# NVlabs/curobo

Hardware: NVIDIA H100
Metric: rollout_cost_grad_evals_per_sec (higher is better)
Workload: dtype f32

## Files before the change

curobo_b200/csrc/cb200_kernels.cu:

```cuda
#include <cuda_runtime.h>
#include <stdio.h>
#include <stdlib.h>
#include <string.h>

#include <algorithm>
#include <cmath>
#include <vector>

#include "../../include/curobo_b200.h"
#include "cb200_blob.h"
#include "cb200_bspline.cuh"
#include "cb200_dynamics.cuh"
#include "cb200_dynamics_tile.cuh"
#include "cb200_launch.h"
#include "cb200_math.cuh"
#include "cb200_mesh.cuh"
#include "cb200_warp.cuh"

using namespace cb200;

namespace {

constexpr int kWarpsPerCta = 8;
constexpr int kMinCtas = 2;
// ... 70 lines not shown
  } else if (s.degree == 5) {
    st = bspline::evaluate<5>(bspline::make_polygon<5>(s.knots, b, d, D, s.n_knots, dt, s.steps, implicit, s.sp, s.sv, s.sa, s.sj, srow, s.gp, s.gv, s.ga, s.gj, grow), h, s.steps);
  } else {
    st = bspline::evaluate<4>(bspline::make_polygon<4>(s.knots, b, d, D, s.n_knots, dt, s.steps, implicit, s.sp, s.sv, s.sa, s.sj, srow, s.gp, s.gv, s.ga, s.gj, grow), h, s.steps);
  }
  return st;
}

template <bool SPLINE>
__device__ __forceinline__ bspline::State4 load_row_state(const FusedArgs &a, int e, int b, int h, int d, int D) {
  if (SPLINE) {
    const bspline::State4 st = spline_row_state(a.spl, b, h, d, D);
    const size_t idx = (size_t)e * D + d;
    if (a.spl.out_p) a.spl.out_p[idx] = st.p;
    if (a.spl.out_v) a.spl.out_v[idx] = st.v;
    if (a.spl.out_a) a.spl.out_a[idx] = st.a;
    if (a.spl.out_j) a.spl.out_j[idx] = st.j;
    return st;
  }
  const size_t idx = (size_t)e * D + d;
  bspline::State4 st;
  st.p = __ldg(a.q + idx);
  st.v = a.vel ? __ldg(a.vel + idx) : 0.0f;
  st.a = a.acc ? __ldg(a.acc + idx) : 0.0f;
  st.j = a.jerk ? __ldg(a.jerk + idx) : 0.0f;
  return st;
}

__device__ __forceinline__ float seed_dt(const FusedArgs &a, int b) {
  if (a.spl.knots != nullptr) return __ldg(a.spl.traj_dt + __ldg(a.spl.goal_idx + b));
  return a.dt ? __ldg(a.dt + b) : 1.0f;
}

__device__ __forceinline__ float cspace_dof(const FusedArgs &a, const RobotView &rv, int e, int b, int h, int d,
                                            const bspline::State4 &st, float &gp) {
  const float qd = st.p;
  const cb200_rollout_cfg &c = a.cfg;
  const int D = rv.D;
  const float *lim = rv.limits;
  float cost = 0.0f;
  gp = 0.0f;
  if (c.cspace_type == 1) {
    bound_cost(qd, lim[d], lim[D + d], c.cspace_activation[0], c.cspace_weight[0], cost, gp);
    cspace_target_term(a, b, h, d, D, qd, cost, gp);
  } else if (c.cspace_type == 2) {
    const size_t idx = (size_t)e * D + d;
    const float dt = seed_dt(a, b);
    float wb[5], wr[5];
#pragma unroll
    for (int i = 0; i < 5; ++i) {
      wb[i] = c.cspace_weight[i];
      wr[i] = c.cspace_reg[i];
    }
    const float dt2 = dt * dt, dt3 = dt2 * dt;
    if (c.retime_weights) {
      wb[1] = dt * wb[1];
      wb[2] = dt2 * wb[2];
      wb[3] = dt3 * wb[3];
    }
    if (c.retime_regularization_weights) {
      wr[0] = dt * wr[0];
      wr[1] = dt2 * wr[1];
      wr[2] = dt3 * wr[2];
      wr[4] = dt * wr[4];
    }
    const float v = st.v, ac = st.a, jk = st.j;
    float gv = 0.0f, ga = 0.0f, gj = 0.0f;
    bound_cost(qd, lim[d], lim[D + d], c.cspace_activation[0], wb[0], cost, gp);
    bound_cost(v, lim[2 * D + d], lim[3 * D + d], c.cspace_activation[1], wb[1], cost, gv);
    bound_cost(ac, lim[4 * D + d], lim[5 * D + d], c.cspace_activation[2], wb[2], cost, ga);
    bound_cost(jk, lim[6 * D + d], lim[7 * D + d], c.cspace_activation[3], wb[3], cost, gj);
    cspace_target_term(a, b, h, d, D, qd, cost, gp);
    l2_reg(v, wr[0], cost, gv);
    l2_reg(ac, wr[1], cost, ga);
    l2_reg(jk, wr[2], cost, gj);
    if (a.grad_vel) a.grad_vel[idx] = gv;
    if (a.grad_acc) a.grad_acc[idx] = ga;
    if (a.grad_jerk) a.grad_jerk[idx] = gj;
  }
  return cost;
}

template <bool SPLINE, int W = 32>
__device__ __forceinline__ void row_phase_a(const FusedArgs &a, const RobotView &rv, const EvalSmem &es, int lane, int e,
                                            int b, int h, float &cs_cost, float &pose_c) {
  const cb200_rollout_cfg &cfg = a.cfg;
  const int D = rv.D, S = rv.S, L = rv.L;
  cs_cost = 0.0f;
  #pragma unroll 1
  for (int d = lane; d < D; d += W) {
    const bspline::State4 st = load_row_state<SPLINE>(a, e, b, h, d, D);
    es.qv[d] = st.p;
    float gp;
    const float c = cspace_dof(a, rv, e, b, h, d, st, gp);
    es.gqv[d] = gp;
    cs_cost += c;
    if (a.cspace_cost) a.cspace_cost[(size_t)e * D + d] = c;
  }
  row_sync<W>();
  warp_fk<W>(rv, es, lane);
  warp_spheres<W>(rv, es, lane, a.robot_spheres ? reinterpret_cast<float4 *>(a.robot_spheres) + (size_t)e * S : nullptr,
                  row_sphere_cfg(a, b, S));
  pose_c = 0.0f;
  const bool do_pose = (a.goal_position != nullptr);
  #pragma unroll 1
  for (int t = lane; t < L; t += W) {
    const float *T = es.cumul + 12 * rv.tool_map[t];
    const V3 p = mk3(T[3], T[7], T[11]);
    const Q4 qt = quat_from_transform(T);
    if (a.link_pos) {
      float *o = a.link_pos + ((size_t)e * L + t) * 3;
      o[0] = p.x;
      o[1] = p.y;
      o[2] = p.z;
    }
    if (a.link_quat) *reinterpret_cast<float4 *>(a.link_quat + ((size_t)e * L + t) * 4) = make_float4(qt.w, qt.x, qt.y, qt.z);
    float *pg = es.pose_g + 8 * t;
    pg[0] = pg[1] = pg[2] = pg[4] = pg[5] = pg[6] = 0.0f;
    if (do_pose) {
      const int gi = a.idxs_goal ? __ldg(a.idxs_goal + b) : 0;
      const bool term = !(h < a.H - 1 && a.H > 1);
      const float *axes = term ? a.pose_axes_t : a.pose_axes_nt;
      const float *tol = term ? a.pose_tol_t : a.pose_tol_nt;
      const size_t go = ((size_t)gi * L + t) * cfg.num_goalset;
      const PoseOut po = tool_pose_cost(p, qt, a.goal_position + go * 3, a.goal_quat + go * 4, cfg.num_goalset,
                                        cfg.pose_weight[0], cfg.pose_weight[1], axes, t,
                                        tol != nullptr ? __ldg(tol + 2 * t) : 0.0f,
                                        tol != nullptr ? __ldg(tol + 2 * t + 1) : 0.0f, cfg.pose_rotation_method);
      const V3 om = quat_grad_to_omega(qt, po.gq_w, po.gq_x, po.gq_y, po.gq_z);
      pg[0] = po.g_pos.x;
      pg[1] = po.g_pos.y;
      pg[2] = po.g_pos.z;
      pg[4] = om.x;
      pg[5] = om.y;
      pg[6] = om.z;
      pose_c += po.pos_cost + po.rot_cost;
      if (a.pose_cost) {
        a.pose_cost[((size_t)e * L + t) * 2] = po.pos_cost;
        a.pose_cost[((size_t)e * L + t) * 2 + 1] = po.rot_cost;
      }
      if (a.pose_goalset_idx) a.pose_goalset_idx[(size_t)e * L + t] = po.goal_idx;
    }
  }
  row_sync<W>();
}

struct RowB1 {
  float self_c, fmax, scene_c;
  int bi, bj, nnz;
};

__device__ __forceinline__ float4 mesh_terms(const MeshSet *ms, float eta, float w, V3 c, float r, int env, bool sweep, bool has_prev,
                                          V3 prev, bool has_next, V3 next) {
  const CuboidSet no_cuboids{};
  const VoxelSet no_voxels{};
  V3 g = mk3(0, 0, 0);
  const float cost = sweep ? sphere_scene_swept<4>(c, r, eta, w, has_prev, prev, has_next, next, no_cuboids, no_voxels, env, g, ms)
                           : sphere_scene_discrete<4>(c, r, eta, w, no_cuboids, no_voxels, env, g, ms);
  return make_float4(g.x, g.y, g.z, cost);
}

template <bool SWEEP, int SCENE, bool CULL2 = true, int W = 32>
__device__ __forceinline__ RowB1 row_phase_b1(const FusedArgs &a, const RobotView &rv, const EvalSmem &es, int lane, int e,
                                              int b, const float4 *prev_sph, const float4 *next_sph) {
  const cb200_rollout_cfg &cfg = a.cfg;
  const int S = rv.S;
  RowB1 r{0.0f, 0.0f, 0.0f, 0, 0, 0};
  if (cfg.self_weight > 0.0f && rv.P > 0) {
    r.fmax = (rv.n_lp > 0) ? warp_self_collision_tiles<true, CULL2, W>(rv, es, lane, r.bi, r.bj)
                           : warp_self_collision_pairs<W>(es.gsph, rv.pairs, rv.P, lane, r.bi, r.bj);
    r.self_c = (r.fmax > 0.0f) ? 0.5f * cfg.self_weight * r.fmax : 0.0f;
  }
  if (a.self_cost && lane == 0) a.self_cost[e] = r.self_c;
  row_sync<W>();
  const bool do_scene = SCENE != 0 && cfg.scene_weight > 0.0f;
  const int env = (a.env_query_idx != nullptr) ? __ldg(a.env_query_idx + b) : 0;
  const float sdt = (SWEEP && cfg.use_speed_metric && (a.dt != nullptr || a.spl.knots != nullptr))
                        ? (a.spl.knots != nullptr ? __ldg(a.spl.traj_dt + __ldg(a.spl.goal_idx)) : __ldg(a.dt))
                        : 0.0f;
  int ce = 0, ncub = 0;
  bool cull = false;
  if ((SCENE & 1) && do_scene && (!(SCENE & 4) || a.cuboids.inv_pose != nullptr)) {
    ce = env < a.cuboids.num_envs ? env : 0;
    ncub = a.cuboids.count[ce];
    if (ncub > a.cuboids.max_n) ncub = a.cuboids.max_n;
    cull = !SWEEP && rv.n_lp > 0 && ncub <= 32;
    if (cull) {
#pragma unroll 1
      for (int ca = lane; ca < rv.n_cl; ca += W) {
        const float4 cb = rv.cl_bound_scene[ca];
        uint32_t mask = 0u;
        if (cb.w >= 0.0f) {
          const float *Tk = es.cumul + 12 * rv.cl_link[ca];
          const V3 cw = mk3(Tk[0] * cb.x + Tk[1] * cb.y + Tk[2] * cb.z + Tk[3], Tk[4] * cb.x + Tk[5] * cb.y + Tk[6] * cb.z + Tk[7],
                            Tk[8] * cb.x + Tk[9] * cb.y + Tk[10] * cb.z + Tk[11]);
#pragma unroll 1
          for (int i = 0; i < ncub; ++i) {
            const int kk = ce * a.cuboids.max_n + i;
            if (a.cuboids.enable[kk] != 1) continue;
            const ObsFrame f = load_obs_frame(a.cuboids.inv_pose + 8 * kk);
            const SdfGrad sg = cuboid_sdf_grad(to_obstacle(f, cw), ldgf(a.cuboids.dims + 4 * kk), ldgf(a.cuboids.dims + 4 * kk + 1),
                                               ldgf(a.cuboids.dims + 4 * kk + 2));
            if (sg.sdf < cb.w + cfg.scene_activation) mask |= (1u << i);
          }
        }
        es.cmask[ca] = mask;
      }
      row_sync<W>();
    }
// ... 36 lines not shown
            const float4 m = mesh_terms(&a.meshes, cfg.scene_activation, cfg.scene_weight, cen, sp.w, env, false, false, cen, false, cen);
            c += m.w;
            g = g + mk3(m.x, m.y, m.z);
          }
        }
      } else {
        V3 pv = cen, nx = cen;
        if (prev_sph != nullptr) {
          const float4 t = prev_sph[s];
          pv = mk3(t.x, t.y, t.z);
        }
        if (next_sph != nullptr) {
          const float4 t = next_sph[s];
          nx = mk3(t.x, t.y, t.z);
        }
        c = sphere_scene_swept<SCENE & 3>(cen, sp.w, cfg.scene_activation, cfg.scene_weight, prev_sph != nullptr, pv,
                                          next_sph != nullptr, nx, a.cuboids, a.voxels, env, g);
        if (SCENE & 4) {
          const float4 m = mesh_terms(&a.meshes, cfg.scene_activation, cfg.scene_weight, cen, sp.w, env, true, prev_sph != nullptr,
                                      pv, next_sph != nullptr, nx);
          c += m.w;
          g = g + mk3(m.x, m.y, m.z);
        }
        if (cfg.use_speed_metric && prev_sph != nullptr && next_sph != nullptr) speed_metric(pv, cen, nx, sdt, c, g);
      }
    }
    es.gsph[s] = make_float4(g.x, g.y, g.z, 0.0f);
    r.nnz += (g.x != 0.0f || g.y != 0.0f || g.z != 0.0f) ? 1 : 0;
    r.scene_c += c;
    if (a.scene_cost) a.scene_cost[(size_t)e * S + s] = c;
  }
  row_sync<W>();
  r.nnz = (int)row_reduce<W, 0>((unsigned)r.nnz) + 2;
  return r;
}

template <bool SMALL = false, int W = 32>
__device__ __forceinline__ void row_phase_b2(const FusedArgs &a, const RobotView &rv, const EvalSmem &es,
                                             const unsigned char *smem_blob, int lane, int e, const RowB1 &r,
                                             float cs_cost, float pose_c) {
  if (r.fmax > 0.0f && lane == 0) {
    const float4 pi = es.sph[r.bi], pj = es.sph[r.bj];
    const float w = a.cfg.self_weight;
    float4 gi = es.gsph[r.bi], gj = es.gsph[r.bj];
    const float gx = w * (pj.x - pi.x), gy = w * (pj.y - pi.y), gz = w * (pj.z - pi.z);
    gi.x += gx;
    gi.y += gy;
    gi.z += gz;
    gj.x -= gx;
    gj.y -= gy;
    gj.z -= gz;
    es.gsph[r.bi] = gi;
    es.gsph[r.bj] = gj;
  }
  row_sync<W>();
  float *gq = a.grad_q + (size_t)e * rv.D;
  if (!warp_fk_backward_sparse<SMALL, W>(rv, es, lane, gq, r.nnz)) warp_fk_backward_cold<W>(smem_blob, a.blob, es.cumul, lane, gq);
  const float tot = warp_sum<W>(cs_cost + pose_c + r.scene_c) + r.self_c;
  if (lane == 0) a.cost[e] = tot;
  row_sync<W>();
}

template <int SCENE, bool SPLINE, int MINB = kMinCtas, int ROWS = 1>
__global__ void __launch_bounds__(kWarpsPerCta * 32, MINB) rollout_fused_kernel(const __grid_constant__ FusedArgs a) {
  static_assert(ROWS == 1 || (ROWS == 2 && MINB == 3 && !SPLINE), "paired rows: arm build only");
  constexpr int W = 32 / ROWS;
  CB200_EXTERN_SHARED __align__(128) unsigned char smem[];
  __shared__ unsigned long long mbar;
  stage_blob_to_smem(smem, a.blob, (uint32_t)a.blob_smem_bytes, &mbar);
  const int warp = threadIdx.x >> 5, lane = threadIdx.x & (W - 1), nwarps = blockDim.x >> 5;
  const int half = ROWS == 1 ? 0 : (int)(threadIdx.x >> 4) & 1;
  const bool leader = (threadIdx.x & 31) == 0;
  float *base = reinterpret_cast<float *>(smem + a.blob_smem_bytes) + (size_t)(warp * ROWS + half) * a.eval_floats;
  const int N = a.B * a.H;
  const int stride = gridDim.x * nwarps;
  int u = blockIdx.x * nwarps + warp;
  while (u * ROWS < N) {
    const int e = u * ROWS + half;
    if (ROWS == 1 || e < N) {
      int b = e, h = 0;
      if (a.H != 1) {
        b = e / a.H;
        h = e - b * a.H;
      }
      const RobotView rv = make_robot_view(smem, a.blob);
      const EvalSmem es = carve_eval_smem(base, rv.nl, rv.D, rv.S, rv.L, rv.n_cl);
      float cs_cost = 0.0f, pose_c = 0.0f;
      row_phase_a<SPLINE, W>(a, rv, es, lane, e, b, h, cs_cost, pose_c);
      const RowB1 r = row_phase_b1<false, SCENE, MINB != 3, W>(a, rv, es, lane, e, b, nullptr, nullptr);
      row_phase_b2<MINB == 3, W>(a, rv, es, smem, lane, e, r, cs_cost, pose_c);
    }
    if (a.work_counter != nullptr) {
      int nxt = 0;
      if (leader) nxt = stride + atomicAdd(a.work_counter, 1);
      u = __shfl_sync(kFull, nxt, 0);
    } else {
      u += stride;
    }
  }
  if (a.work_counter != nullptr && leader) {
    __threadfence();
    if (atomicAdd(a.work_counter + 1, 1) == stride - 1) {
      a.work_counter[0] = 0;
      a.work_counter[1] = 0;
    }
  }
}

constexpr int kBigWarps = 16;

template <int SCENE, bool SMALL = false>
__device__ __forceinline__ RowB1 row_phase_b1_list(const FusedArgs &a, const RobotView &rv, const EvalSmem &es, int lane, int e,
                                                   int b, int &n_list, bool &dense) {
  const cb200_rollout_cfg &cfg = a.cfg;
  const int S = rv.S;
  RowB1 r{0.0f, 0.0f, 0.0f, 0, 0, 0};
  n_list = 0;
  dense = false;
  if (cfg.self_weight > 0.0f && rv.P > 0) {
    r.fmax = warp_self_collision_tiles<false, !SMALL>(rv, es, lane, r.bi, r.bj);
    r.self_c = (r.fmax > 0.0f) ? 0.5f * cfg.self_weight * r.fmax : 0.0f;
  }
  if (a.self_cost && lane == 0) a.self_cost[e] = r.self_c;
  __syncwarp();
  const bool do_scene = SCENE != 0 && cfg.scene_weight > 0.0f;
  const int env = (a.env_query_idx != nullptr) ? __ldg(a.env_query_idx + b) : 0;
  int ce = 0, ncub = 0;
  bool cull = false;
  if ((SCENE & 1) && do_scene && (!(SCENE & 4) || a.cuboids.inv_pose != nullptr)) {
    ce = env < a.cuboids.num_envs ? env : 0;
    ncub = a.cuboids.count[ce];
    if (ncub > a.cuboids.max_n) ncub = a.cuboids.max_n;
// ... 1422 lines not shown
      if (d > best) {
        best = d;
        arg = i;
      }
    }
    return best;
  };
  int arg;
  double best_R = farthest(c, arg), best_c[3] = {c[0], c[1], c[2]};
  for (int it = 1; it <= 200; ++it) {
    const double R = farthest(c, arg);
    if (R < best_R) {
      best_R = R;
      for (int k = 0; k < 3; ++k) best_c[k] = c[k];
    }
    const double dx = bx[arg] - c[0], dy = by[arg] - c[1], dz = bz[arg] - c[2];
    const double d = std::sqrt(dx * dx + dy * dy + dz * dz);
    if (d < 1e-12) break;
    const double mv = std::min(R / (it + 1.0), d) / d;
    c[0] += dx * mv;
    c[1] += dy * mv;
    c[2] += dz * mv;
  }
  const double Rf = farthest(best_c, arg);
  out[0] = (float)best_c[0];
  out[1] = (float)best_c[1];
  out[2] = (float)best_c[2];
  double cr[3] = {(double)out[0], (double)out[1], (double)out[2]};
  const double Rr = farthest(cr, arg);
  out[3] = (float)(std::max(Rf, Rr) * (1.0 + 1e-4) + 1e-5);
}

static thread_local int g_last_variant = 0;

extern "C" {

int cb200_abi_version(void) { return CB200_ABI_VERSION; }
int cb200_last_rollout_variant(void) { return g_last_variant; }
int cb200_sm_arch(void) { return 90; }
const char *cb200_error_string(int err) { return cudaGetErrorString((cudaError_t)err); }

int cb200_device_info(int device, int *sm_count, int *max_smem_optin) {
  cudaError_t e = cudaDeviceGetAttribute(sm_count, cudaDevAttrMultiProcessorCount, device);
  if (e != cudaSuccess) return ret(e);
  return ret(cudaDeviceGetAttribute(max_smem_optin, cudaDevAttrMaxSharedMemoryPerBlockOptin, device));
}

int cb200_kinematics_forward_spheres(float *link_pos, float *link_quat, float *batch_robot_spheres,
                                     float *batch_center_of_mass, float *global_cumul_mat, const float *joint_vec,
                                     const float *fixed_transform, const float *robot_spheres,
                                     const float *link_masses_com, const int8_t *joint_map_type,
                                     const int16_t *joint_map, const int16_t *link_map, const int16_t *tool_frame_map,
                                     const int16_t *link_sphere_map, const float *joint_offset_map,
                                     const int32_t *env_query_idx, int num_envs, int batch_size, int horizon,
                                     int n_joints, int num_spheres, int num_links, int n_tool_frames,
                                     int write_global_cumul, int compute_com, cb200_stream_t stream) {
  CB200_DEVICE_GUARD(joint_vec);
  if (batch_size < 0 || num_links < 1 || horizon < 1) return ret(cudaErrorInvalidValue);
  if (compute_com != 0 && (batch_center_of_mass == nullptr || link_masses_com == nullptr)) return ret(cudaErrorInvalidValue);
  if (batch_size == 0) return ret(cudaSuccess);
  KinFwdArgs a{link_pos, link_quat, batch_robot_spheres, global_cumul_mat, joint_vec, fixed_transform, robot_spheres,
               joint_offset_map, joint_map_type, joint_map, link_map, tool_frame_map, link_sphere_map, env_query_idx,
               num_envs, batch_size, horizon, n_joints, num_spheres, num_links, n_tool_frames, write_global_cumul,
               link_masses_com, batch_center_of_mass};
  const size_t smem = (size_t)kWarpsPerCta * num_links * 12 * sizeof(float);
  void (*kern)(const KinFwdArgs) = compute_com != 0 ? kin_forward_kernel<true> : kin_forward_kernel<false>;
  if (smem > 48 * 1024) {
    cudaError_t e = cudaFuncSetAttribute(kern, cudaFuncAttributeMaxDynamicSharedMemorySize, (int)smem);
    if (e != cudaSuccess) return ret(e);
  }
  const int grid = persistent_grid(kern, kWarpsPerCta * 32, smem, (batch_size + kWarpsPerCta - 1) / kWarpsPerCta);
// ... 408 lines not shown
          lps.push_back((uint32_t)a | ((uint32_t)b << 16));
          covered += (long long)(cl_start[a + 1] - cl_start[a]) * (cl_start[b + 1] - cl_start[b]);
        }
      }
      ok = ok && covered == P && (int)lps.size() <= lp_cap(sz);
    }
    if (ok) {
      std::sort(lps.begin(), lps.end(), [](uint32_t x, uint32_t y) {
        return ((x & 0xffffu) != (y & 0xffffu)) ? (x & 0xffffu) < (y & 0xffffu) : (x >> 16) < (y >> 16);
      });
      BlobHeader *hh = reinterpret_cast<BlobHeader *>(o);
      hh->n_cl = n_cl;
      hh->n_lp = (int32_t)lps.size();
      int16_t *cll = reinterpret_cast<int16_t *>(o + h.off_cl_link);
      int16_t *cls = reinterpret_cast<int16_t *>(o + h.off_cl_start);
      float *clb = reinterpret_cast<float *>(o + h.off_cl_bound);
      for (int a = 0; a < n_cl; ++a) {
        cll[a] = (int16_t)cl_link[a];
        cls[a] = (int16_t)cl_start[a];
        bounding_ball(link_spheres, sphere_padding, cl_start[a], cl_start[a + 1], clb + 4 * a, n_cfg, S);
        bounding_ball(link_spheres, nullptr, cl_start[a], cl_start[a + 1],
                      reinterpret_cast<float *>(o + h.off_cl_bound_scene) + 4 * a, n_cfg, S);
      }
      cls[n_cl] = (int16_t)S;
      memcpy(o + h.off_lp, lps.data(), lps.size() * 4);
      for (int s0 = 0; s0 < S; ++s0) o[h.off_sph_cl + s0] = (unsigned char)cl_of_sphere[s0];
    }
  }
  return total;
}

int cb200_rollout_cost_grad(const cb200_rollout_cfg *cfg, const cb200_rollout_io *io, cb200_stream_t stream) {
  CB200_DEVICE_GUARD((io != nullptr ? io->cost : nullptr));
  if (cfg == nullptr || io == nullptr || io->robot_blob == nullptr || io->cost == nullptr || io->grad_q == nullptr ||
      io->batch_size < 0 || io->horizon < 1)
    return ret(cudaErrorInvalidValue);
  const cb200_spline_input *sp = io->spline;
  if (sp == nullptr && io->q == nullptr) return ret(cudaErrorInvalidValue);
  int spline_steps = 0;
  if (sp != nullptr) {
    if (sp->knots == nullptr || sp->start_position == nullptr || sp->start_velocity == nullptr ||
        sp->start_acceleration == nullptr || sp->start_jerk == nullptr || sp->start_idx == nullptr ||
        sp->goal_idx == nullptr || sp->traj_dt == nullptr || sp->use_implicit_goal_state == nullptr ||
        sp->goal_position == nullptr || sp->goal_velocity == nullptr || sp->goal_acceleration == nullptr ||
        sp->goal_jerk == nullptr || sp->n_knots < 1 || sp->degree < 3 || sp->degree > 5)
      return ret(cudaErrorInvalidValue);
    spline_steps = (io->horizon - 1) / (sp->n_knots + sp->degree + 1);
    if (sp->grad_knots != nullptr &&
        (io->grad_vel == nullptr || io->grad_acc == nullptr || io->grad_jerk == nullptr || io->horizon - 1 < 5 ||
         spline_steps < 1 || spline_steps > 32))
      return ret(cudaErrorInvalidValue);
  }
  if (io->goal_position != nullptr && (io->goal_quat == nullptr || cfg->num_goalset < 1)) return ret(cudaErrorInvalidValue);
  const long long N = (long long)io->batch_size * io->horizon;
  if (N == 0) return ret(cudaSuccess);
  if (io->robot_blob_host == nullptr) return ret(cudaErrorInvalidValue);
  BlobHeader cached_hdr;
  memcpy(&cached_hdr, io->robot_blob_host, sizeof(BlobHeader));
  if (cached_hdr.magic != kBlobMagic || cached_hdr.total_bytes != io->robot_blob_bytes) return ret(cudaErrorInvalidValue);
  const BlobHeader &h = cached_hdr;
  FusedArgs a{};
  a.cfg = *cfg;
  a.q = io->q;
  a.vel = io->vel;
  a.acc = io->acc;
  a.jerk = io->jerk;
// ... 145 lines not shown
      long long g = (long long)d.sm_count * bp.per_sm;
      const long long need_ctas = (N + bp.nw - 1) / bp.nw;
      if (g > need_ctas) g = need_ctas;
      g_last_variant = CB200_VARIANT_BIG;
      CB200_LAUNCH(bk, (int)(g < 1 ? 1 : g), bp.nw * 32, bp.smem, (cudaStream_t)stream, a);
      return finish();
    }
  }
  const size_t halo_bytes = traj ? (size_t)2 * h.S * sizeof(float4) : 0;
  if (io->dynamics != nullptr) {
    const cb200_dynamics_params *dp = io->dynamics;
    if (dp->link_masses_com == nullptr || dp->link_inertias == nullptr || dp->gravity == nullptr || !traj ||
        cfg->cspace_type != 2 || spline || a.vel == nullptr || a.acc == nullptr)
      return ret(cudaErrorInvalidValue);
    a.dyn = FusedArgs::Dyn{dp->link_masses_com, dp->link_inertias, dp->gravity};
    using DynKernelT = void (*)(const FusedArgs, const int);
    static DynKernelT const traj_dyn[4] = {rollout_traj_dyn_kernel<0>, rollout_traj_dyn_kernel<1>, rollout_traj_dyn_kernel<2>,
                                           rollout_traj_dyn_kernel<3>};
    DynKernelT dk = traj_dyn[scene];
    const cudaError_t e = cached_plan(PlanKey{(const void *)dk, d.ordinal, (size_t)h.smem_bytes + halo_bytes, a.eval_floats,
                                              io->horizon, h.nl, h.D},
                                      d, plan_dyn, p);
    if (e != cudaSuccess) return ret(e);
    if (p.nw == 0) return ret(cudaErrorInvalidConfiguration);
    long long grid_ll = (long long)d.sm_count * p.per_sm;
    const long long need_ctas = (long long)io->batch_size * ((io->horizon + p.R - 1) / p.R);
    if (grid_ll > need_ctas) grid_ll = need_ctas;
    g_last_variant = CB200_VARIANT_TRAJ_DYN;
    CB200_LAUNCH(dk, (int)(grid_ll < 1 ? 1 : grid_ll), p.nw * 32, p.smem, (cudaStream_t)stream, a, p.R);
    return finish();
  }
  KernelT kern;
  int rows_per_warp = 1;
  bool arm = false;
  if (traj) {
    static KernelT const traj_full[2][4] = {
        {rollout_traj_kernel<0, false>, rollout_traj_kernel<1, false>, rollout_traj_kernel<2, false>, rollout_traj_kernel<3, false>},
        {rollout_traj_kernel<0, true>, rollout_traj_kernel<1, true>, rollout_traj_kernel<2, true>, rollout_traj_kernel<3, true>}};
    static KernelT const traj_small[2][4] = {
        {rollout_traj_kernel<0, false, true>, rollout_traj_kernel<1, false, true>, rollout_traj_kernel<2, false, true>,
         rollout_traj_kernel<3, false, true>},
        {rollout_traj_kernel<0, true, true>, rollout_traj_kernel<1, true, true>, rollout_traj_kernel<2, true, true>,
         rollout_traj_kernel<3, true, true>}};
    if (arm_sized) kern = mesh ? rollout_traj_kernel<7, false, true> : traj_small[spline][scene];
    else kern = mesh ? rollout_traj_kernel<7, false> : traj_full[spline][scene];
  } else if (!spline && !mesh && arm_sized) {
    static KernelT const arm_rows[4] = {rollout_fused_kernel<0, false, 3>, rollout_fused_kernel<1, false, 3>,
                                        rollout_fused_kernel<2, false, 3>, rollout_fused_kernel<3, false, 3>};
    static KernelT const arm_pairs[2] = {rollout_fused_kernel<0, false, 3, 2>, rollout_fused_kernel<1, false, 3, 2>};
    const int pairs_env = env_int("CB200_ARM_PAIRS", -1);
    const bool pairs = h.nl <= 16 && (scene & 2) == 0 &&
                       (pairs_env >= 0 ? pairs_env != 0 : 2LL * N >= 3LL * d.sm_count * 3 * kWarpsPerCta);
    kern = pairs ? arm_pairs[scene] : arm_rows[scene];
    rows_per_warp = pairs ? 2 : 1;
    arm = true;
  } else {
    static KernelT const fused[2][4] = {
        {rollout_fused_kernel<0, false>, rollout_fused_kernel<1, false>, rollout_fused_kernel<2, false>, rollout_fused_kernel<3, false>},
        {rollout_fused_kernel<0, true>, rollout_fused_kernel<1, true>, rollout_fused_kernel<2, true>, rollout_fused_kernel<3, true>}};
    kern = mesh ? rollout_fused_kernel<7, false> : fused[spline][scene];
  }
  const cudaError_t e =
      cached_plan(PlanKey{(const void *)kern, d.ordinal, (size_t)h.smem_bytes + halo_bytes, rows_per_warp * a.eval_floats,
                          traj ? io->horizon : 0, 0, 0},
                  d, [](const PlanKey &k, size_t limit) { return plan_warps(k, limit, kWarpsPerCta); }, p);
  if (e != cudaSuccess) return ret(e);
  if (p.nw == 0) return ret(cudaErrorInvalidConfiguration);
  const int nw = p.nw;
  a.work_counter = counter;
  if (traj && (long long)io->batch_size * ((io->horizon + nw - 1) / nw) > 0x3fffffffLL) a.work_counter = nullptr;
  long long grid_ll = (long long)d.sm_count * p.per_sm;
  const long long units = (N + rows_per_warp - 1) / rows_per_warp;
  const long long need_ctas = traj ? (long long)io->batch_size * ((io->horizon + nw - 1) / nw) : (units + nw - 1) / nw;
  if (grid_ll > need_ctas) grid_ll = need_ctas;
  const int grid = (int)(grid_ll < 1 ? 1 : grid_ll);
  if (need_ctas <= grid_ll) a.work_counter = nullptr;
  g_last_variant = traj ? CB200_VARIANT_TRAJ : (arm ? CB200_VARIANT_ARM : CB200_VARIANT_STANDARD);
  CB200_LAUNCH(kern, grid, nw * 32, p.smem, (cudaStream_t)stream, a);
  return finish();
}

}
```

curobo_b200/csrc/cb200_warp.cuh:

```cuda
#pragma once
#include "cb200_blob.h"
#include "cb200_math.cuh"

namespace cb200 {

constexpr unsigned kFull = 0xffffffffu;

struct RobotView {
  int nl, D, S, L, P, n_levels;
  const float *fixed;
  const float *joff;
  const int16_t *link_map;
  const int16_t *joint_map;
  const int8_t *joint_type;
  const int16_t *tool_map;
  const float4 *spheres;
  const int16_t *sph_link;
  const float *padding;
  const int16_t *link_sph_off;
  const int16_t *link_sph_idx;
  const int16_t *level_off;
  const int16_t *level_links;
  const unsigned long long *anc_mask;
  const int16_t *jl_off;
// ... 168 lines not shown
  if (W == 32) return __shfl_xor_sync(kFull, v, o);
#ifdef CB200_SIMT_EMULATION
  const int me = threadIdx.x & 15;
  return half_exchange(v, [me, o](const unsigned long long *s) { return s[me ^ o]; });
#else
  return __shfl_xor_sync(row_mask<W>(), v, o);
#endif
}
template <int W, int OP>
__device__ __forceinline__ unsigned row_reduce(unsigned v) {
  if (W == 32) return OP == 0 ? __reduce_add_sync(kFull, v) : OP == 1 ? __reduce_min_sync(kFull, v) : __reduce_max_sync(kFull, v);
#ifdef CB200_SIMT_EMULATION
  return half_exchange(v, [](const unsigned long long *s) {
    unsigned r = (unsigned)s[0];
    for (int i = 1; i < 16; ++i) {
      const unsigned x = (unsigned)s[i];
      r = OP == 0 ? r + x : OP == 1 ? (x < r ? x : r) : (x > r ? x : r);
    }
    return (unsigned long long)r;
  });
#else
  const unsigned m = row_mask<W>();
  return OP == 0 ? __reduce_add_sync(m, v) : OP == 1 ? __reduce_min_sync(m, v) : __reduce_max_sync(m, v);
#endif
}

template <int W = 32>
__device__ __forceinline__ float warp_sum(float v) {
#pragma unroll
  for (int o = W / 2; o > 0; o >>= 1) v += row_shfl_xor<W>(v, o);
  return v;
}

template <int W = 32>
__device__ __forceinline__ void warp_fk_compose(const RobotView &rv, const EvalSmem &es, int lane);
template <int W = 32>
__device__ __forceinline__ void warp_fk(const RobotView &rv, const EvalSmem &es, int lane) {
  const bool scratch = rv.S * 4 >= rv.nl * 12;
  float *loc = scratch ? reinterpret_cast<float *>(es.sph) : es.cumul;
  #pragma unroll 1
  for (int l = lane; l < rv.nl; l += W) {
    int jt = rv.joint_type[l];
    float th = 0.0f;
    if (jt >= 0) th = rv.joff[2 * l] * es.qv[rv.joint_map[l]] + rv.joff[2 * l + 1];
    local_link_transform(rv.fixed + 12 * l, jt, th, (l == 0 ? es.cumul : loc) + 12 * l);
  }
  row_sync<W>();
  warp_fk_compose<W>(rv, es, lane);
}

template <int W>
__device__ __forceinline__ void warp_fk_compose(const RobotView &rv, const EvalSmem &es, int lane) {
  const bool scratch = rv.S * 4 >= rv.nl * 12;
  const float *loc = scratch ? reinterpret_cast<const float *>(es.sph) : es.cumul;
  const int half = lane >> 4, k = lane & 15;
  const bool lane_ok = k < 12;
  const uint32_t row_off = (uint32_t)(k >> 2) * 16u, col_off = (uint32_t)(k & 3) * 4u, k_off = (uint32_t)k * 4u;
  const float cw = ((k & 3) == 3) ? 1.0f : 0.0f;
  unsigned char *cumb = reinterpret_cast<unsigned char *>(es.cumul);
  const unsigned char *locb = reinterpret_cast<const unsigned char *>(loc);
#pragma unroll 1
  for (int st = 0; st < rv.n_fk_steps; ++st) {
#pragma unroll
    for (int pass = 0; pass < 32 / W; ++pass) {
      const int sub = W == 32 ? half : pass;
      const uint32_t w = rv.fk_sched[2 * st + sub];
      const uint32_t l_off = w & 0xffffu, p_off = w >> 16;
      if (W == 16 && l_off == 0xffffu) continue;
      const bool act = lane_ok && (l_off != 0xffffu);
      float out = 0.0f;
      if (act) {
        const float4 pr = *reinterpret_cast<const float4 *>(cumb + p_off + row_off);
        const float *Lm = reinterpret_cast<const float *>(locb + l_off + col_off);
        out = pr.x * Lm[0] + pr.y * Lm[4] + pr.z * Lm[8] + cw * pr.w;
      }
      if (!scratch) row_sync<W>();
      if (act) *reinterpret_cast<float *>(cumb + l_off + k_off) = out;
      row_sync<W>();
    }
  }
}

template <int W = 32>
__device__ __forceinline__ void warp_spheres(const RobotView &rv, const EvalSmem &es, int lane, float4 *out_global,
                                             const float4 *cfg_spheres = nullptr) {
  #pragma unroll 1
  for (int s = lane; s < rv.S; s += W) {
// ... 612 lines not shown
```

curobo_b200/lib.py:

```python
from __future__ import annotations

import ctypes as C
import os
from typing import Optional

_LIB: Optional[C.CDLL] = None

c_f = C.c_void_p
c_p = C.c_void_p


class CuboidSet(C.Structure):
    _fields_ = [("dims", C.c_void_p), ("inv_pose", C.c_void_p), ("enable", C.c_void_p), ("count", C.c_void_p),
                ("max_n", C.c_int32), ("num_envs", C.c_int32)]


class VoxelSet(C.Structure):
    _fields_ = [("params", C.c_void_p), ("inv_pose", C.c_void_p), ("enable", C.c_void_p), ("count", C.c_void_p),
                ("features", C.c_void_p), ("n_voxels_per_layer", C.c_int32), ("max_n", C.c_int32),
                ("num_envs", C.c_int32), ("max_dist", C.c_float), ("mip", C.c_void_p), ("mip_stride", C.c_int32)]


class MeshSet(C.Structure):
    _fields_ = [("nodes", C.c_void_p), ("triangles", C.c_void_p), ("node_offset", C.c_void_p), ("triangle_offset", C.c_void_p),
# ... 19 lines not shown
    _fields_ = [("knots", c_p), ("start_position", c_p), ("start_velocity", c_p), ("start_acceleration", c_p),
                ("start_jerk", c_p), ("goal_position", c_p), ("goal_velocity", c_p), ("goal_acceleration", c_p),
                ("goal_jerk", c_p), ("start_idx", c_p), ("goal_idx", c_p), ("traj_dt", c_p),
                ("use_implicit_goal_state", c_p), ("n_knots", C.c_int32), ("degree", C.c_int32), ("grad_knots", c_p),
                ("out_position", c_p), ("out_velocity", c_p), ("out_acceleration", c_p), ("out_jerk", c_p),
                ("out_dt", c_p)]


class DynamicsParams(C.Structure):
    _fields_ = [("link_masses_com", c_p), ("link_inertias", c_p), ("gravity", c_p)]


class RolloutIO(C.Structure):
    _fields_ = [("q", c_p), ("vel", c_p), ("acc", c_p), ("jerk", c_p), ("dt", c_p),
                ("robot_blob", c_p), ("robot_blob_host", c_p), ("robot_blob_bytes", C.c_int32),
                ("cuboids", C.POINTER(CuboidSet)), ("voxels", C.POINTER(VoxelSet)), ("env_query_idx", c_p),
                ("goal_position", c_p), ("goal_quat", c_p), ("idxs_goal", c_p),
                ("pose_axes_terminal", c_p), ("pose_axes_non_terminal", c_p),
                ("pose_tol_terminal", c_p), ("pose_tol_non_terminal", c_p),
                ("cost", c_p), ("grad_q", c_p), ("self_cost", c_p), ("scene_cost", c_p), ("pose_cost", c_p),
                ("cspace_cost", c_p), ("grad_vel", c_p), ("grad_acc", c_p), ("grad_jerk", c_p),
                ("link_pos", c_p), ("link_quat", c_p), ("robot_spheres", c_p), ("pose_goalset_idx", c_p),
                ("batch_size", C.c_int32), ("horizon", C.c_int32), ("spline", C.POINTER(SplineInput)),
                ("dynamics", C.POINTER(DynamicsParams)),
                ("cspace_target", c_p), ("idxs_cspace_target", c_p), ("cspace_target_dof_weight", c_p),
                ("sphere_configs", c_p), ("num_sphere_configs", C.c_int32), ("work_counter", c_p),
                ("meshes", C.POINTER(MeshSet))]


_I = C.c_int
_SIGS = {
    "cb200_abi_version": ([], _I),
    "cb200_last_rollout_variant": ([], _I),
    "cb200_sm_arch": ([], _I),
    "cb200_error_string": ([_I], C.c_char_p),
    "cb200_device_info": ([_I, C.POINTER(_I), C.POINTER(_I)], _I),
    "cb200_kinematics_forward_spheres": ([c_p] * 16 + [_I] * 9 + [c_p], _I),
    "cb200_kinematics_backward": ([c_p] * 22 + [_I] * 9 + [c_p], _I),
    "cb200_self_collision_distance": ([c_p] * 10 + [_I] * 8 + [c_p], _I),
    "cb200_sphere_obstacle_collision": ([c_p] * 3 + [C.POINTER(CuboidSet), C.POINTER(VoxelSet)] + [c_p] * 3 + [_I] * 4 + [c_p], _I),
    "cb200_swept_sphere_obstacle_collision": ([c_p] * 3 + [C.POINTER(CuboidSet), C.POINTER(VoxelSet)] + [c_p] * 3 + [_I, c_p] + [_I] * 4 + [c_p], _I),
    "cb200_tool_pose_distance": ([c_p] * 16 + [_I] * 5 + [c_p], _I),
    "cb200_cspace_state_cost": ([c_p] * 25 + [_I] * 6 + [c_p], _I),
    "cb200_cspace_position_cost": ([c_p] * 19 + [_I] * 4 + [c_p], _I),
    "cb200_bspline_forward": ([c_p] * 18 + [_I] * 5 + [c_p], _I),
    "cb200_bspline_single_dt": ([c_p] * 20 + [_I] * 5 + [c_p], _I),
    "cb200_bspline_backward": ([c_p] * 8 + [_I] * 5 + [c_p], _I),
    "cb200_lbfgs_step": ([c_p] * 8 + [C.c_float] + [_I] * 4 + [c_p] * 3 + [_I, c_p, _I, _I, c_p], _I),
    "cb200_line_search": ([c_p] * 5 + [_I, C.c_float, C.c_float] + [c_p] * 13 + [C.c_float, C.c_float] + [_I] * 5 + [c_p], _I),
    "cb200_voxel_mip_block": ([], _I),
    "cb200_voxel_mip_stride": ([c_p, _I], C.c_int64),
    "cb200_voxel_build_mip": ([C.POINTER(VoxelSet), c_p], _I),
    "cb200_rnea_forward": ([c_p] * 15 + [_I] * 4 + [c_p, c_p], _I),
    "cb200_rnea_backward": ([c_p] * 17 + [_I] * 4 + [c_p, c_p], _I),
    "cb200_pba3d": ([c_p, c_p, _I, _I, _I, _I, c_p], _I),
    "cb200_sphere_mesh_collision": ([c_p, c_p, c_p, C.POINTER(MeshSet), c_p, c_p, c_p, _I, c_p, _I, _I, _I, _I, _I, _I, c_p], _I),
    "cb200_edt_unsigned_distance": ([c_p, c_p, _I, _I, _I, C.c_float, C.c_float, c_p], _I),
    "cb200_esdf_seed_sites": ([c_p, c_p, _I, _I, _I, C.c_float, C.c_float, c_p], _I),
    "cb200_esdf_signed_distance": ([c_p, c_p, c_p, c_p, _I, _I, _I, C.c_float, C.c_float, c_p], _I),
    "cb200_esdf_seed_sites_gather": ([c_p, c_p, _I, _I, _I, C.c_float, C.c_float, C.POINTER(C.c_float), c_p], _I),
    "cb200_tsdf_integrate_depth": ([c_p, _I, _I, _I, C.c_float, C.POINTER(C.c_float), _I, c_p, c_p, c_p, c_p, _I, _I, C.c_float,
                                    C.c_float, C.c_float, c_p], _I),
    "cb200_tsdf_combined_sdf": ([c_p, c_p, c_p, C.c_longlong, C.c_float, c_p], _I),
    "cb200_tsdf_stamp_cuboids": ([c_p, _I, _I, _I, C.c_float, C.POINTER(C.c_float), C.c_float, C.POINTER(CuboidSet), _I, c_p], _I),
    "cb200_robot_blob_bytes": ([C.POINTER(RobotSizes)], C.c_int64),
    "cb200_pack_robot_blob": ([c_p, C.c_int64, C.POINTER(RobotSizes)] + [c_p] * 15, C.c_int64),
# ... 41 lines not shown
```

include/curobo_b200.h:

```cpp
#ifndef CUROBO_B200_H
#define CUROBO_B200_H

#include <stdint.h>

#ifdef __cplusplus
extern "C" {
#endif

typedef struct CUstream_st *cb200_stream_t;

#define CB200_ABI_VERSION 6

int cb200_abi_version(void);
int cb200_sm_arch(void);
const char *cb200_error_string(int err);
#define CB200_VARIANT_NONE 0
#define CB200_VARIANT_STANDARD 1
#define CB200_VARIANT_ARM 2
#define CB200_VARIANT_BIG 4
#define CB200_VARIANT_TEAM2 5
#define CB200_VARIANT_TEAM4 6
#define CB200_VARIANT_TRAJ 7
#define CB200_VARIANT_TRAJ_DYN 8
int cb200_last_rollout_variant(void);

int cb200_kinematics_forward_spheres(
    float *link_pos, float *link_quat, float *batch_robot_spheres, float *batch_center_of_mass,
    float *global_cumul_mat, const float *joint_vec, const float *fixed_transform,
    const float *robot_spheres, const float *link_masses_com, const int8_t *joint_map_type,
    const int16_t *joint_map, const int16_t *link_map, const int16_t *tool_frame_map,
    const int16_t *link_sphere_map, const float *joint_offset_map, const int32_t *env_query_idx,
    int num_envs, int batch_size, int horizon, int n_joints, int num_spheres, int num_links,
    int n_tool_frames, int write_global_cumul, int compute_com, cb200_stream_t stream);

int cb200_kinematics_backward(
    float *grad_out, const float *grad_nlinks_pos, const float *grad_nlinks_quat,
    const float *grad_spheres, const float *grad_center_of_mass, const float *batch_center_of_mass,
    const float *grad_jacobian, const float *global_cumul_mat, const float *robot_spheres,
    const float *link_masses_com, const int16_t *link_map, const int16_t *joint_map,
    const int8_t *joint_map_type, const int16_t *tool_frame_map, const int16_t *link_sphere_map,
    const int16_t *link_chain_data, const int16_t *link_chain_offsets, const int16_t *joint_links_data,
    const int16_t *joint_links_offsets, const uint8_t *joint_affects_endeffector,
    const float *joint_offset_map, const int32_t *env_query_idx, int num_envs, int batch_size,
    int horizon, int n_joints, int num_spheres, int num_links, int n_tool_frames, int compute_com,
    int compute_jacobian_grad, cb200_stream_t stream);

int cb200_self_collision_distance(
    float *out_distance, float *out_vec, float *pair_distance, uint8_t *sparse_index,
    const float *robot_spheres, const float *sphere_padding, const float *weight,
    const int16_t *pair_locations, float *block_batch_max_value, int16_t *block_batch_max_index,
    int num_blocks_per_batch, int max_threads_per_block, int batch_size, int horizon, int nspheres,
    int num_collision_pairs, int store_pair_distance, int compute_grad, cb200_stream_t stream);

typedef struct {
  const float *dims;
  const float *inv_pose;
  const uint8_t *enable;
// ... 257 lines not shown
```

Measured before the change: 258.5 million.

## Add lean paired-row arm kernel variant with one-pass FK compose for plain configs

```diff
diff --git a/curobo_b200/csrc/cb200_kernels.cu b/curobo_b200/csrc/cb200_kernels.cu
--- a/curobo_b200/csrc/cb200_kernels.cu
+++ b/curobo_b200/csrc/cb200_kernels.cu
@@ -126,6 +126,7 @@
   return a.dt ? __ldg(a.dt + b) : 1.0f;
 }
 
+template <bool LEAN = false>
 __device__ __forceinline__ float cspace_dof(const FusedArgs &a, const RobotView &rv, int e, int b, int h, int d,
                                             const bspline::State4 &st, float &gp) {
   const float qd = st.p;
@@ -136,8 +137,8 @@
   gp = 0.0f;
   if (c.cspace_type == 1) {
     bound_cost(qd, lim[d], lim[D + d], c.cspace_activation[0], c.cspace_weight[0], cost, gp);
-    cspace_target_term(a, b, h, d, D, qd, cost, gp);
-  } else if (c.cspace_type == 2) {
+    if (!LEAN) cspace_target_term(a, b, h, d, D, qd, cost, gp);
+  } else if (!LEAN && c.cspace_type == 2) {
     const size_t idx = (size_t)e * D + d;
     const float dt = seed_dt(a, b);
     float wb[5], wr[5];
@@ -175,9 +176,47 @@
   return cost;
 }
 
-template <bool SPLINE, int W = 32>
+enum RowPhase { kPhCspace, kPhFkLocal, kPhFkCompose, kPhSpheres, kPhToolPose, kPhSelf, kPhScene, kPhJt, kPhRowCost, kNumPhases };
+#ifdef CB200_PHASE_CLOCKS
+constexpr int kSpanWarps = 16384;
+__device__ unsigned long long g_phase_cycles[kNumPhases + 1];
+__device__ unsigned long long g_warp_span[2 * kSpanWarps];
+__shared__ unsigned s_phase[kNumPhases + 2];
+__device__ __forceinline__ unsigned long long global_ns() {
+  unsigned long long t;
+  asm volatile("mov.u64 %0, %%globaltimer;" : "=l"(t));
+  return t;
+}
+struct PhaseClock {
+  unsigned t;
+  bool lead;
+  __device__ void start(bool row_lead) {
+    lead = row_lead;
+    t = (unsigned)clock();
+  }
+  __device__ void mark(int p) {
+    const unsigned n = (unsigned)clock();
+    if (lead) atomicAdd(&s_phase[p], n - t);
+    t = n;
+  }
+  __device__ void row_done() {
+    if (lead) atomicAdd(&s_phase[kNumPhases], 1u);
+  }
+};
+#else
+struct PhaseClock {
+  __device__ void start(bool) {}
+  __device__ void mark(int) {}
+  __device__ void row_done() {}
+};
+#endif
+__device__ __forceinline__ void phase_mark(PhaseClock *pc, int p) {
+  if (pc != nullptr) pc->mark(p);
+}
+
+template <bool SPLINE, int W = 32, bool LEAN = false>
 __device__ __forceinline__ void row_phase_a(const FusedArgs &a, const RobotView &rv, const EvalSmem &es, int lane, int e,
-                                            int b, int h, float &cs_cost, float &pose_c) {
+                                            int b, int h, float &cs_cost, float &pose_c, PhaseClock *pc = nullptr) {
   const cb200_rollout_cfg &cfg = a.cfg;
   const int D = rv.D, S = rv.S, L = rv.L;
   cs_cost = 0.0f;
@@ -186,15 +225,22 @@
     const bspline::State4 st = load_row_state<SPLINE>(a, e, b, h, d, D);
     es.qv[d] = st.p;
     float gp;
-    const float c = cspace_dof(a, rv, e, b, h, d, st, gp);
+    const float c = cspace_dof<LEAN>(a, rv, e, b, h, d, st, gp);
     es.gqv[d] = gp;
     cs_cost += c;
     if (a.cspace_cost) a.cspace_cost[(size_t)e * D + d] = c;
   }
   row_sync<W>();
-  warp_fk<W>(rv, es, lane);
-  warp_spheres<W>(rv, es, lane, a.robot_spheres ? reinterpret_cast<float4 *>(a.robot_spheres) + (size_t)e * S : nullptr,
-                  row_sphere_cfg(a, b, S));
+  phase_mark(pc, kPhCspace);
+  warp_fk_local<W>(rv, es, lane);
+  row_sync<W>();
+  phase_mark(pc, kPhFkLocal);
+  warp_fk_compose<W, LEAN>(rv, es, lane);
+  phase_mark(pc, kPhFkCompose);
+  if (LEAN) warp_spheres<W>(rv, es, lane, nullptr);
+  else warp_spheres<W>(rv, es, lane, a.robot_spheres ? reinterpret_cast<float4 *>(a.robot_spheres) + (size_t)e * S : nullptr,
+                       row_sphere_cfg(a, b, S));
+  phase_mark(pc, kPhSpheres);
   pose_c = 0.0f;
   const bool do_pose = (a.goal_position != nullptr);
   #pragma unroll 1
@@ -202,13 +248,13 @@
     const float *T = es.cumul + 12 * rv.tool_map[t];
     const V3 p = mk3(T[3], T[7], T[11]);
     const Q4 qt = quat_from_transform(T);
-    if (a.link_pos) {
+    if (!LEAN && a.link_pos) {
       float *o = a.link_pos + ((size_t)e * L + t) * 3;
       o[0] = p.x;
       o[1] = p.y;
       o[2] = p.z;
     }
-    if (a.link_quat) *reinterpret_cast<float4 *>(a.link_quat + ((size_t)e * L + t) * 4) = make_float4(qt.w, qt.x, qt.y, qt.z);
+    if (!LEAN && a.link_quat) *reinterpret_cast<float4 *>(a.link_quat + ((size_t)e * L + t) * 4) = make_float4(qt.w, qt.x, qt.y, qt.z);
     float *pg = es.pose_g + 8 * t;
     pg[0] = pg[1] = pg[2] = pg[4] = pg[5] = pg[6] = 0.0f;
     if (do_pose) {
@@ -237,6 +283,7 @@
     }
   }
   row_sync<W>();
+  phase_mark(pc, kPhToolPose);
 }
 
 struct RowB1 {
@@ -254,9 +301,9 @@
   return make_float4(g.x, g.y, g.z, cost);
 }
 
-template <bool SWEEP, int SCENE, bool CULL2 = true, int W = 32>
+template <bool SWEEP, int SCENE, bool CULL2 = true, int W = 32, bool LEAN = false>
 __device__ __forceinline__ RowB1 row_phase_b1(const FusedArgs &a, const RobotView &rv, const EvalSmem &es, int lane, int e,
-                                              int b, const float4 *prev_sph, const float4 *next_sph) {
+                                              int b, const float4 *prev_sph, const float4 *next_sph, PhaseClock *pc = nullptr) {
   const cb200_rollout_cfg &cfg = a.cfg;
   const int S = rv.S;
   RowB1 r{0.0f, 0.0f, 0.0f, 0, 0, 0};
@@ -267,8 +314,9 @@
   }
   if (a.self_cost && lane == 0) a.self_cost[e] = r.self_c;
   row_sync<W>();
+  phase_mark(pc, kPhSelf);
   const bool do_scene = SCENE != 0 && cfg.scene_weight > 0.0f;
-  const int env = (a.env_query_idx != nullptr) ? __ldg(a.env_query_idx + b) : 0;
+  const int env = (!LEAN && a.env_query_idx != nullptr) ? __ldg(a.env_query_idx + b) : 0;
   const float sdt = (SWEEP && cfg.use_speed_metric && (a.dt != nullptr || a.spl.knots != nullptr))
                         ? (a.spl.knots != nullptr ? __ldg(a.spl.traj_dt + __ldg(a.spl.goal_idx)) : __ldg(a.dt))
                         : 0.0f;
@@ -371,13 +419,14 @@
   }
   row_sync<W>();
   r.nnz = (int)row_reduce<W, 0>((unsigned)r.nnz) + 2;
+  phase_mark(pc, kPhScene);
   return r;
 }
 
 template <bool SMALL = false, int W = 32>
 __device__ __forceinline__ void row_phase_b2(const FusedArgs &a, const RobotView &rv, const EvalSmem &es,
                                              const unsigned char *smem_blob, int lane, int e, const RowB1 &r,
-                                             float cs_cost, float pose_c) {
+                                             float cs_cost, float pose_c, PhaseClock *pc = nullptr) {
   if (r.fmax > 0.0f && lane == 0) {
     const float4 pi = es.sph[r.bi], pj = es.sph[r.bj];
     const float w = a.cfg.self_weight;
@@ -395,22 +444,37 @@
   row_sync<W>();
   float *gq = a.grad_q + (size_t)e * rv.D;
   if (!warp_fk_backward_sparse<SMALL, W>(rv, es, lane, gq, r.nnz)) warp_fk_backward_cold<W>(smem_blob, a.blob, es.cumul, lane, gq);
+  phase_mark(pc, kPhJt);
   const float tot = warp_sum<W>(cs_cost + pose_c + r.scene_c) + r.self_c;
   if (lane == 0) a.cost[e] = tot;
   row_sync<W>();
 }
 
-template <int SCENE, bool SPLINE, int MINB = kMinCtas, int ROWS = 1>
+template <int SCENE, bool SPLINE, int MINB = kMinCtas, int ROWS = 1, bool LEAN = false>
 __global__ void __launch_bounds__(kWarpsPerCta * 32, MINB) rollout_fused_kernel(const __grid_constant__ FusedArgs a) {
   static_assert(ROWS == 1 || (ROWS == 2 && MINB == 3 && !SPLINE), "paired rows: arm build only");
+  static_assert(!LEAN || ROWS == 2, "lean build: paired arm rows only");
   constexpr int W = 32 / ROWS;
   CB200_EXTERN_SHARED __align__(128) unsigned char smem[];
   __shared__ unsigned long long mbar;
+#ifdef CB200_PHASE_CLOCKS
+  const int span = blockIdx.x * (blockDim.x >> 5) + (threadIdx.x >> 5);
+  if ((threadIdx.x & 31) == 0 && span < kSpanWarps) g_warp_span[2 * span] = global_ns();
+  if (threadIdx.x < kNumPhases + 2) s_phase[threadIdx.x] = 0u;
+  __syncthreads();
+#endif
   stage_blob_to_smem(smem, a.blob, (uint32_t)a.blob_smem_bytes, &mbar);
   const int warp = threadIdx.x >> 5, lane = threadIdx.x & (W - 1), nwarps = blockDim.x >> 5;
   const int half = ROWS == 1 ? 0 : (int)(threadIdx.x >> 4) & 1;
   const bool leader = (threadIdx.x & 31) == 0;
   float *base = reinterpret_cast<float *>(smem + a.blob_smem_bytes) + (size_t)(warp * ROWS + half) * a.eval_floats;
+  PhaseClock pc;
+#ifdef CB200_PHASE_CLOCKS
+  PhaseClock *const pcp = &pc;
+#else
+  PhaseClock *const pcp = nullptr;
+#endif
+  pc.start(lane == 0);
   const int N = a.B * a.H;
   const int stride = gridDim.x * nwarps;
   int u = blockIdx.x * nwarps + warp;
@@ -418,16 +482,17 @@
     const int e = u * ROWS + half;
     if (ROWS == 1 || e < N) {
       int b = e, h = 0;
-      if (a.H != 1) {
+      if (!LEAN && a.H != 1) {
         b = e / a.H;
         h = e - b * a.H;
       }
       const RobotView rv = make_robot_view(smem, a.blob);
       const EvalSmem es = carve_eval_smem(base, rv.nl, rv.D, rv.S, rv.L, rv.n_cl);
       float cs_cost = 0.0f, pose_c = 0.0f;
-      row_phase_a<SPLINE, W>(a, rv, es, lane, e, b, h, cs_cost, pose_c);
-      const RowB1 r = row_phase_b1<false, SCENE, MINB != 3, W>(a, rv, es, lane, e, b, nullptr, nullptr);
-      row_phase_b2<MINB == 3, W>(a, rv, es, smem, lane, e, r, cs_cost, pose_c);
+      row_phase_a<SPLINE, W, LEAN>(a, rv, es, lane, e, b, h, cs_cost, pose_c, pcp);
+      const RowB1 r = row_phase_b1<false, SCENE, MINB != 3, W, LEAN>(a, rv, es, lane, e, b, nullptr, nullptr, pcp);
+      row_phase_b2<MINB == 3, W>(a, rv, es, smem, lane, e, r, cs_cost, pose_c, pcp);
+      pc.row_done();
     }
     if (a.work_counter != nullptr) {
       int nxt = 0;
@@ -436,7 +501,19 @@
     } else {
       u += stride;
     }
-  }
+    phase_mark(pcp, kPhRowCost);
+  }
+#ifdef CB200_PHASE_CLOCKS
+  __syncwarp();
+  if (leader) {
+    if (span < kSpanWarps) g_warp_span[2 * span + 1] = global_ns();
+    __threadfence_block();
+    if (atomicAdd(&s_phase[kNumPhases + 1], 1u) == (unsigned)nwarps - 1u) {
+      __threadfence_block();
+      for (int i = 0; i <= kNumPhases; ++i) atomicAdd(&g_phase_cycles[i], (unsigned long long)atomicAdd(&s_phase[i], 0u));
+    }
+  }
+#endif
   if (a.work_counter != nullptr && leader) {
     __threadfence();
     if (atomicAdd(a.work_counter + 1, 1) == stride - 1) {
@@ -1925,11 +2002,29 @@
 }
 
 static thread_local int g_last_variant = 0;
+static thread_local int g_last_lean = 0;
 
 extern "C" {
 
 int cb200_abi_version(void) { return CB200_ABI_VERSION; }
 int cb200_last_rollout_variant(void) { return g_last_variant; }
+int cb200_last_rollout_lean(void) { return g_last_lean; }
+#ifdef CB200_PHASE_CLOCKS
+int cb200_phase_clocks_reset(void) {
+  static const unsigned long long zeros[2 * kSpanWarps] = {};
+  cudaError_t e = cudaMemcpyToSymbol(g_phase_cycles, zeros, sizeof(g_phase_cycles));
+  if (e == cudaSuccess) e = cudaMemcpyToSymbol(g_warp_span, zeros, sizeof(g_warp_span));
+  return (int)e;
+}
+int cb200_phase_clocks_read(unsigned long long *cycles, unsigned long long *spans, int max_warps) {
+  if (max_warps > kSpanWarps) max_warps = kSpanWarps;
+  cudaError_t e = cudaDeviceSynchronize();
+  if (e == cudaSuccess) e = cudaMemcpyFromSymbol(cycles, g_phase_cycles, sizeof(g_phase_cycles));
+  if (e == cudaSuccess) e = cudaMemcpyFromSymbol(spans, g_warp_span, (size_t)2 * max_warps * sizeof(unsigned long long));
+  return (int)e;
+}
+int cb200_phase_clocks_count(void) { return kNumPhases; }
+#endif
 int cb200_sm_arch(void) { return 90; }
 const char *cb200_error_string(int err) { return cudaGetErrorString((cudaError_t)err); }
 
@@ -2404,6 +2499,7 @@
 
 int cb200_rollout_cost_grad(const cb200_rollout_cfg *cfg, const cb200_rollout_io *io, cb200_stream_t stream) {
   CB200_DEVICE_GUARD((io != nullptr ? io->cost : nullptr));
+  g_last_lean = 0;
   if (cfg == nullptr || io == nullptr || io->robot_blob == nullptr || io->cost == nullptr || io->grad_q == nullptr ||
       io->batch_size < 0 || io->horizon < 1)
     return ret(cudaErrorInvalidValue);
@@ -2615,7 +2711,7 @@
   }
   KernelT kern;
   int rows_per_warp = 1;
-  bool arm = false;
+  bool arm = false, lean_launch = false;
   if (traj) {
     static KernelT const traj_full[2][4] = {
         {rollout_traj_kernel<0, false>, rollout_traj_kernel<1, false>, rollout_traj_kernel<2, false>, rollout_traj_kernel<3, false>},
@@ -2631,10 +2727,15 @@
     static KernelT const arm_rows[4] = {rollout_fused_kernel<0, false, 3>, rollout_fused_kernel<1, false, 3>,
                                         rollout_fused_kernel<2, false, 3>, rollout_fused_kernel<3, false, 3>};
     static KernelT const arm_pairs[2] = {rollout_fused_kernel<0, false, 3, 2>, rollout_fused_kernel<1, false, 3, 2>};
+    static KernelT const arm_lean[2] = {rollout_fused_kernel<0, false, 3, 2, true>, rollout_fused_kernel<1, false, 3, 2, true>};
     const int pairs_env = env_int("CB200_ARM_PAIRS", -1);
     const bool pairs = h.nl <= 16 && (scene & 2) == 0 &&
                        (pairs_env >= 0 ? pairs_env != 0 : 2LL * N >= 3LL * d.sm_count * 3 * kWarpsPerCta);
-    kern = pairs ? arm_pairs[scene] : arm_rows[scene];
+    const bool plain = io->horizon == 1 && cfg->cspace_type != 2 && a.cs_target == nullptr && a.link_pos == nullptr &&
+                       a.link_quat == nullptr && a.robot_spheres == nullptr && a.env_query_idx == nullptr && a.sphere_cfgs == nullptr;
+    const bool lean = pairs && plain && env_int("CB200_ARM_LEAN", 1) != 0;
+    kern = lean ? arm_lean[scene] : pairs ? arm_pairs[scene] : arm_rows[scene];
+    lean_launch = lean;
     rows_per_warp = pairs ? 2 : 1;
     arm = true;
   } else {
@@ -2659,6 +2760,7 @@
   const int grid = (int)(grid_ll < 1 ? 1 : grid_ll);
   if (need_ctas <= grid_ll) a.work_counter = nullptr;
   g_last_variant = traj ? CB200_VARIANT_TRAJ : (arm ? CB200_VARIANT_ARM : CB200_VARIANT_STANDARD);
+  g_last_lean = lean_launch ? 1 : 0;
   CB200_LAUNCH(kern, grid, nw * 32, p.smem, (cudaStream_t)stream, a);
   return finish();
 }
diff --git a/curobo_b200/csrc/cb200_warp.cuh b/curobo_b200/csrc/cb200_warp.cuh
--- a/curobo_b200/csrc/cb200_warp.cuh
+++ b/curobo_b200/csrc/cb200_warp.cuh
@@ -224,10 +224,10 @@
   return v;
 }
 
-template <int W = 32>
+template <int W = 32, bool ONE_PASS = false>
 __device__ __forceinline__ void warp_fk_compose(const RobotView &rv, const EvalSmem &es, int lane);
 template <int W = 32>
-__device__ __forceinline__ void warp_fk(const RobotView &rv, const EvalSmem &es, int lane) {
+__device__ __forceinline__ void warp_fk_local(const RobotView &rv, const EvalSmem &es, int lane) {
   const bool scratch = rv.S * 4 >= rv.nl * 12;
   float *loc = scratch ? reinterpret_cast<float *>(es.sph) : es.cumul;
   #pragma unroll 1
@@ -237,14 +237,49 @@
     if (jt >= 0) th = rv.joff[2 * l] * es.qv[rv.joint_map[l]] + rv.joff[2 * l + 1];
     local_link_transform(rv.fixed + 12 * l, jt, th, (l == 0 ? es.cumul : loc) + 12 * l);
   }
+}
+template <int W = 32, bool ONE_PASS = false>
+__device__ __forceinline__ void warp_fk(const RobotView &rv, const EvalSmem &es, int lane) {
+  warp_fk_local<W>(rv, es, lane);
   row_sync<W>();
-  warp_fk_compose<W>(rv, es, lane);
-}
-
-template <int W>
+  warp_fk_compose<W, ONE_PASS>(rv, es, lane);
+}
+
+template <int W, bool ONE_PASS>
 __device__ __forceinline__ void warp_fk_compose(const RobotView &rv, const EvalSmem &es, int lane) {
   const bool scratch = rv.S * 4 >= rv.nl * 12;
   const float *loc = scratch ? reinterpret_cast<const float *>(es.sph) : es.cumul;
+  if (ONE_PASS) {
+    static_assert(!ONE_PASS || W == 16, "one compose pass per step: half-warp rows");
+    const int sub = lane >= 6 ? 1 : 0, j = lane - 6 * sub;
+    const bool lane_ok = lane < 12;
+    const int r = j >> 1, c = 2 * (j & 1);
+    const uint32_t row_off = (uint32_t)r * 16u, col_off = (uint32_t)c * 4u, k_off = (uint32_t)(4 * r + c) * 4u;
+    const float cw0 = c + 0 == 3 ? 1.0f : 0.0f, cw1 = c + 1 == 3 ? 1.0f : 0.0f;
+    unsigned char *cumb = reinterpret_cast<unsigned char *>(es.cumul);
+    const unsigned char *locb = reinterpret_cast<const unsigned char *>(loc);
+#pragma unroll 1
+    for (int st = 0; st < rv.n_fk_steps; ++st) {
+      const uint32_t w = rv.fk_sched[2 * st + sub];
+      const uint32_t l_off = w & 0xffffu, p_off = w >> 16;
+      const bool act = lane_ok && (l_off != 0xffffu);
+      float out0 = 0.0f, out1 = 0.0f;
+      if (act) {
+        const float4 pr = *reinterpret_cast<const float4 *>(cumb + p_off + row_off);
+        const float *Lm = reinterpret_cast<const float *>(locb + l_off + col_off);
+        out0 = pr.x * Lm[0] + pr.y * Lm[4] + pr.z * Lm[8] + cw0 * pr.w;
+        out1 = pr.x * Lm[1] + pr.y * Lm[5] + pr.z * Lm[9] + cw1 * pr.w;
+      }
+      if (!scratch) row_sync<W>();
+      if (act) {
+        float *o = reinterpret_cast<float *>(cumb + l_off + k_off);
+        o[0] = out0;
+        o[1] = out1;
+      }
+      row_sync<W>();
+    }
+    return;
+  }
   const int half = lane >> 4, k = lane & 15;
   const bool lane_ok = k < 12;
   const uint32_t row_off = (uint32_t)(k >> 2) * 16u, col_off = (uint32_t)(k & 3) * 4u, k_off = (uint32_t)k * 4u;
diff --git a/curobo_b200/lib.py b/curobo_b200/lib.py
--- a/curobo_b200/lib.py
+++ b/curobo_b200/lib.py
@@ -75,6 +75,7 @@
 _SIGS = {
     "cb200_abi_version": ([], _I),
     "cb200_last_rollout_variant": ([], _I),
+    "cb200_last_rollout_lean": ([], _I),
     "cb200_sm_arch": ([], _I),
     "cb200_error_string": ([_I], C.c_char_p),
     "cb200_device_info": ([_I, C.POINTER(_I), C.POINTER(_I)], _I),
diff --git a/include/curobo_b200.h b/include/curobo_b200.h
--- a/include/curobo_b200.h
+++ b/include/curobo_b200.h
@@ -23,6 +23,7 @@
 #define CB200_VARIANT_TRAJ 7
 #define CB200_VARIANT_TRAJ_DYN 8
 int cb200_last_rollout_variant(void);
+int cb200_last_rollout_lean(void);
 
 int cb200_kinematics_forward_spheres(
     float *link_pos, float *link_quat, float *batch_robot_spheres, float *batch_center_of_mass,
```

Result: faster. 267.7 million, median of 6 (+3.5%).
